# zixinz990/quaternion-mpc

Hardware: AMD Instinct MI355X
Metric: MPC QP solves/sec (Go1, 12 forces, N=10) (higher is better)
Workload: dtype f64

## Files before the change

### quaternion-mpc_amd/csrc/qmpc_wform.h

```cpp
#pragma once

namespace qmpc {


struct LayoutW {
  int GK, WR, SLW;
};
constexpr int kGK = 27;
template <int NL = 4>
__host__ __device__ inline size_t wform_slice(int N, bool sl_global = false) {
  return ((size_t)N * (13 * 12 + 21 * NL + kGK + (sl_global ? 18 * NL : 0)) + 1 + 1) & ~(size_t)1;
}
template <int NL = 4>
__host__ __device__ inline Layout make_layout_w(int N, LayoutW* W, bool kd_global = false, bool sl_global = false, bool cv = false,
                                                bool full = false) {
  Layout L;
  int o = 0;
  auto take = [&](int n) { int r = o; o += n; return r; };
  constexpr int nu = 3 * NL, nc = 6 * NL, nl = NL;
  L.cst = take(NL == 4 ? 64 : 80);
  L.bw0 = take(3 * nu);
  L.refp = take(13);
  L.uref = take(nu);
  L.X = take((N + 1) * 13);
// ... 301 lines not shown
  bool c12;
  template <int NL = 4, int MD = WM_QUAT>
  __device__ __forceinline__ void init(const DevParams& P, const Layout& L, int lane) {
    const int N = P.N;
    const int c = lane & 15, g = lane >> 4;
    co.init(P, c);
    const int zs = L.cst + kZeroSlotsT<NL>();
    const bool c35 = (c >= 3 && c < 6), c911 = (c >= 9 && c < 12);
    c12 = c == 12;
    const int abN = L.AB + kAB * (N - 1);
    ix_w = c35 ? abN + 18 + (c - 3) : zs;   st_w = c35 ? kAB : 0;
    ix_a = c35 ? abN + (c - 3) : (c911 ? abN + 9 + (c - 9) : zs);   st_a = (c35 || c911) ? kAB : 0;
    sel[0] = (g == 3) ? 1.0 : 0.0;
    sel[1] = (g == 0) ? 1.0 : 0.0;
    sel[2] = (g == 1) ? 1.0 : 0.0;
    const double m1 = P.h * (P.hh * (1.0 / P.mass)), m2 = P.h * (1.0 / P.mass);
#pragma unroll
    for (int e = 0; e < 3; ++e) {
      const int r = 4 * e + g;
      const bool phi = (r >= 3 && r < 6);
      double v = 0.0;
      if (c < 6) {
        if (r < 3) v = (r == c) ? m1 : 0.0;
        else if (r >= 6 && r < 9) v = (r - 6 == c) ? m2 : 0.0;
        else if (r >= 9) v = (r - 9 == c - 3) ? P.h : 0.0;
      }
      Mc[e] = v;
      if (MD == WM_CONVEX) qadd[e] = (c < 12 && r == c) ? P.Q[cvperm(r < 12 ? r : 0)] : 0.0;
      else qadd[e] = (c < 12 && r == c && !phi) ? P.Q[(r < 3) ? r : r + 1] : 0.0;
      const bool xv = (MD == WM_CONVEX) ? c12 : ((phi && c35) || c12);
      const int xo = c12 ? 9 + r : 3 * (r - 3) + (c - 3);
      xoffN[e] = xv ? xo : -1;
      ix_x[e] = xv ? L.XT + kXT * (N - 1) + xo : zs;
      st_x[e] = xv ? kXT : 0;
    }
#pragma unroll
    for (int e = 0; e < 2; ++e) {
      const int r = 4 * e + g;
      const bool phi = (r >= 3 && r < 6);
      Nc[e] = (r < 3 && c == r + 6) ? P.h : ((phi && r == c) ? -1.0 : 0.0);
      const bool gv = r < 6 && (c < 6 || c12);
      const int go = c12 ? 21 + r : S6I(r < 6 ? r : 0, c < 6 ? c : 0);
      ix_g[e] = gv ? kGK * (N - 1) + go : kGK * N;
      st_g[e] = gv ? kGK : 0;
      kwo[e] = (r < 6 && c < 13) ? 13 * r + c : -1;
    }
  }
};
__device__ __forceinline__ void fma_bcast345_x2(double r[2], const double x[2], const double sh[2], double cs, const double m[3]) {
  asm("v_fmac_f64 %0, %4, %5\n\t"
      "v_fmac_f64 %1, %4, %6\n\t"
      "v_fmac_f64_dpp %0, %2, %7 row_newbcast:3 row_mask:0xf bank_mask:0xf\n\t"
      "v_fmac_f64_dpp %1, %3, %7 row_newbcast:3 row_mask:0xf bank_mask:0xf\n\t"
      "v_fmac_f64_dpp %0, %2, %8 row_newbcast:4 row_mask:0xf bank_mask:0xf\n\t"
      "v_fmac_f64_dpp %1, %3, %8 row_newbcast:4 row_mask:0xf bank_mask:0xf\n\t"
      "v_fmac_f64_dpp %0, %2, %9 row_newbcast:5 row_mask:0xf bank_mask:0xf\n\t"
      "v_fmac_f64_dpp %1, %3, %9 row_newbcast:5 row_mask:0xf bank_mask:0xf"
      : "+v"(r[0]), "+v"(r[1])
      : "v"(x[0]), "v"(x[1]), "v"(cs), "v"(sh[0]), "v"(sh[1]), "v"(m[0]), "v"(m[1]), "v"(m[2]));
}
__device__ __forceinline__ void fma_bcast345_x3(double r[3], const double x[3], const double sh[3], double cs, const double m[3]) {
  asm("v_fmac_f64 %0, %6, %7\n\t"
      "v_fmac_f64 %1, %6, %8\n\t"
      "v_fmac_f64 %2, %6, %9\n\t"
      "v_fmac_f64_dpp %0, %3, %10 row_newbcast:3 row_mask:0xf bank_mask:0xf\n\t"
      "v_fmac_f64_dpp %1, %4, %10 row_newbcast:3 row_mask:0xf bank_mask:0xf\n\t"
      "v_fmac_f64_dpp %2, %5, %10 row_newbcast:3 row_mask:0xf bank_mask:0xf\n\t"
      "v_fmac_f64_dpp %0, %3, %11 row_newbcast:4 row_mask:0xf bank_mask:0xf\n\t"
      "v_fmac_f64_dpp %1, %4, %11 row_newbcast:4 row_mask:0xf bank_mask:0xf\n\t"
      "v_fmac_f64_dpp %2, %5, %11 row_newbcast:4 row_mask:0xf bank_mask:0xf\n\t"
      "v_fmac_f64_dpp %0, %3, %12 row_newbcast:5 row_mask:0xf bank_mask:0xf\n\t"
      "v_fmac_f64_dpp %1, %4, %12 row_newbcast:5 row_mask:0xf bank_mask:0xf\n\t"
      "v_fmac_f64_dpp %2, %5, %12 row_newbcast:5 row_mask:0xf bank_mask:0xf"
      : "+v"(r[0]), "+v"(r[1]), "+v"(r[2])
      : "v"(x[0]), "v"(x[1]), "v"(x[2]), "v"(cs), "v"(sh[0]), "v"(sh[1]), "v"(sh[2]), "v"(m[0]), "v"(m[1]), "v"(m[2]));
}
__device__ __forceinline__ void times_M(const double x[2], const ColOps& co, const double wt[3], double r[2]) {
  double sh[2];
#pragma unroll
  for (int e = 0; e < 2; ++e) {
    r[e] = co.m1c * x[e];
    sh[e] = dpp_mov<0x106>(x[e]);
  }
  fma_bcast345_x2(r, x, sh, co.m2c, wt);
}
__device__ __forceinline__ void times_Abar(const double x[3], const ColOps& co, const double at[3], double r[3]) {
  double sh[3];
#pragma unroll
  for (int e = 0; e < 3; ++e) {
    r[e] = co.keep * x[e];
    sh[e] = dpp_mov<0x116>(x[e]);
  }
  fma_bcast345_x3(r, x, sh, co.hsel, at);
}

template <int J0, bool INV = false>
__device__ __forceinline__ void gj6_pair_step(double M[2], double Rr[2], double pc[2], int c, int g, bool& pd, double* Iv = nullptr) {
  constexpr int ej = J0 >> 2, g0 = J0 & 3, g1 = g0 + 1;
  static_assert((J0 & 1) == 0 && J0 < 6, "pivot pairs (0,1), (2,3), (4,5)");
  const int s0 = (g0 << 4) | c, s1 = (g1 << 4) | c;
  const double m0 = __shfl(M[ej], s0), m1 = __shfl(M[ej], s1);
  const double r0 = __shfl(Rr[ej], s0), r1 = __shfl(Rr[ej], s1);
  double i0 = 0.0, i1 = 0.0;
  if (INV) { i0 = __shfl(Iv[ej], s0); i1 = __shfl(Iv[ej], s1); }
  const double a = read_lane(M[ej], (g0 << 4) | J0), b = read_lane(M[ej], (g0 << 4) | (J0 + 1)),
               d = read_lane(M[ej], (g1 << 4) | (J0 + 1));
  const double det = fma(a, d, -(b * b));
  pd = pd && (a > 0.0) && (det > 0.0);
  const double rd = fast_rcp(det);
  const double ia = a * rd, ib = b * rd, id = d * rd;
#pragma unroll
  for (int e = 0; e < 2; ++e) {
    double c0, c1;
    double bm = M[e], br = Rr[e], bi = INV ? Iv[e] : 0.0;
    if (e == ej) {
      const bool p0 = g == g0, p1 = g == g1;
      constexpr int others = 0xF & ~((1 << g0) | (1 << g1));
      c0 = pc[0] = row_bcast_rows<J0, others>(M[e], pc[0]);
      c1 = pc[1] = row_bcast_rows<J0 + 1, others>(M[e], pc[1]);
      if (p0 || p1) { bm = 0.0; br = 0.0; bi = 0.0; }
    } else {
      c0 = row_bcast<J0>(M[e]);
      c1 = row_bcast<J0 + 1>(M[e]);
    }
    const double f0 = fma(ib, c1, -(id * c0)), f1 = fma(ib, c0, -(ia * c1));
    M[e] = fma(f1, m1, fma(f0, m0, bm));
    Rr[e] = fma(f1, r1, fma(f0, r0, br));
    if (INV) Iv[e] = fma(f1, i1, fma(f0, i0, bi));
  }
}

template <bool PROF, bool REFINE = false, int MD = WM_QUAT>
__device__ inline int backward_pass_w(const DevParams& P, const Layout& L, const BwPat& bp, double* sm, double* KD,
                                      const double* GK, int lane, Prof<PROF>& prof, double* y0out = nullptr) {
  const int N = P.N;
  const int c = lane & 15, g = lane >> 4;
  const double wscale = (MD == WM_CONVEX) ? P.h * P.hh : (0.5 * P.hh) * P.h;
  const ColOps& co = bp.co;
  const double* Mc = bp.Mc;
  const double* Nc = bp.Nc;
  const double* qadd = bp.qadd;
  const double* msel = bp.sel;
  const double* nsel = bp.sel;
  const int* xoffN = bp.xoffN;
  const int* kwo = bp.kwo;
  int ix_w = bp.ix_w, ix_a = bp.ix_a, ix_x[3] = {bp.ix_x[0], bp.ix_x[1], bp.ix_x[2]}, ix_g[2] = {bp.ix_g[0], bp.ix_g[1]};
  const bool rowok1 = kwo[1] >= 0;
  double Pf[3];
  {
    const double* XTk = sm + L.XT + kXT * N;
#pragma unroll
    for (int e = 0; e < 3; ++e) Pf[e] = qadd[e] + ((xoffN[e] >= 0) ? XTk[xoffN[e]] : 0.0);
  }
  bool pd = true;
  const d4 z4 = {0.0, 0.0, 0.0, 0.0};
  double pc01[2] = {(g == 0) ? 1.0 : 0.0, (g == 1) ? 1.0 : 0.0}, pc23[2] = {(g == 2) ? 1.0 : 0.0, (g == 3) ? 1.0 : 0.0};
  struct KnotOps { double wt[3], at[3], gr[2], xt[3]; };
  auto load_head = [&](KnotOps& o) {
#pragma unroll
    for (int t = 0; t < 3; ++t) o.wt[t] = sm[ix_w + 3 * t];
    ix_w -= bp.st_w;
#pragma unroll
    for (int e = 0; e < 2; ++e) { o.gr[e] = GK[ix_g[e]]; ix_g[e] -= bp.st_g[e]; }
  };
  auto load_tail = [&](KnotOps& o) {
#pragma unroll
    for (int t = 0; t < 3; ++t) {
      o.at[t] = sm[ix_a + 3 * t]; o.xt[t] = sm[ix_x[t]];
      ix_x[t] -= bp.st_x[t];
    }
    ix_a -= bp.st_a;
  };
  KnotOps ops;
  load_head(ops);
  for (int k = N - 1; k >= 0; --k) {
    double wt[3], Mf[3], Nf[2], R6f[2];
    const double* at = ops.at;
    const double* xt = ops.xt;
    const double Gf[2] = {ops.gr[0], ops.gr[1]};
#pragma unroll
    for (int t = 0; t < 3; ++t) wt[t] = wscale * ops.wt[t];
    load_tail(ops);
    Mf[0] = fma(msel[0], wt[0], Mc[0]);
    Mf[1] = fma(msel[1], wt[1], fma(msel[2], wt[2], Mc[1]));
    Mf[2] = Mc[2];
    Nf[0] = fma(nsel[0], at[0], Nc[0]);
    Nf[1] = fma(nsel[1], at[1], fma(nsel[2], at[2], Nc[1]));
    R6f[0] = bp.c12 ? Gf[0] : 0.0;
    R6f[1] = bp.c12 ? Gf[1] : 0.0;
    tick_dep(prof, PH_BUILD, Pf[0], Pf[1]);
    double Yp[2];
    {
      const d4 a = mtm3(Mf, Pf, z4);
      Yp[0] = a[0]; Yp[1] = a[1];
    }
    if (y0out && bp.c12) {
      if (g < 4) y0out[6 * k + g] = Yp[0];
      if (g < 2) y0out[6 * k + 4 + g] = Yp[1];
    }
    tick_dep(prof, PH_DRAIN, Yp[0], Yp[1]);
    double S6[2];
    times_M(Yp, co, wt, S6);
    double Cf[2], Qf[2], Wm[2];
    {
      const d4 a = mtm2(Gf, Yp, acc_rows(R6f[0], R6f[1]));
      Cf[0] = a[0]; Cf[1] = a[1];
      const d4 b = mtm2(S6, Cf, z4);
      Qf[0] = b[0]; Qf[1] = b[1];
    }
    times_M(Qf, co, wt, Wm);
    Wm[0] = S6[0] + Wm[0];
    Wm[1] = S6[1] + Wm[1];
    if (k > 0) load_head(ops);
    tick_dep(prof, PH_MFMA, Wm[0], Wm[1]);
    double Iv[2];
    if (REFINE) {
      Iv[0] = (c == g) ? 1.0 : 0.0;
      Iv[1] = (g < 2 && c == 4 + g) ? 1.0 : 0.0;
    }
    double Xf[2];
    gj6_pair_step<0, REFINE>(Wm, Qf, pc01, c, g, pd, Iv);
    gj6_pair_step<2, REFINE>(Wm, Qf, pc23, c, g, pd, Iv);
    gj6_pair_step<4, REFINE>(Wm, Qf, pc01, c, g, pd, Iv);
    Xf[0] = Qf[0];
    Xf[1] = rowok1 ? Qf[1] : 0.0;
    if (REFINE) {
      double nWi[2], T1[2], nr[2], vv[2];
      nWi[0] = Iv[0];
      nWi[1] = (g < 2) ? Iv[1] : 0.0;
      {
        const d4 a = mtm2(S6, Xf, z4);
        T1[0] = a[0]; T1[1] = a[1];
      }
      {
        const d4 ini = {Cf[0] + Xf[0], Cf[1] + Xf[1], 0.0, 0.0};
        const d4 a = mtm2(Gf, T1, ini);
        nr[0] = a[0]; nr[1] = rowok1 ? a[1] : 0.0;
      }
      {
        const d4 a = mtm2(S6, nr, z4);
        vv[0] = a[0]; vv[1] = a[1];
      }
      {
        const d4 ini = {Xf[0], Xf[1], 0.0, 0.0};
        const d4 a = mtm2(nWi, vv, ini);
        Xf[0] = a[0];
        Xf[1] = rowok1 ? a[1] : 0.0;
      }
    }
    tick_dep(prof, PH_SOLVE, Xf[0], Xf[1]);
    double Pi[3];
    {
      const d4 a = mtm2(Yp, Xf, acc_rows(Pf[0], Pf[1], Pf[2]));
      Pi[0] = a[0]; Pi[1] = a[1]; Pi[2] = a[2];
    }
    double Zf[2];
    {
      const d4 a = mtm2(S6, Xf, acc_rows(Yp[0], Yp[1]));
      Zf[0] = a[0]; Zf[1] = a[1];
    }
    double Uf[3];
    times_Abar(Pi, co, at, Uf);
    {
      const d4 a = mtm2(Nf, Uf, acc_rows(Uf[0] + (qadd[0] + xt[0]), Uf[1] + (qadd[1] + xt[1]), Uf[2] + (qadd[2] + xt[2])));
      Pf[0] = a[0]; Pf[1] = a[1]; Pf[2] = a[2];
    }
    {
      double* KDk = KD + 156 * k;
#pragma unroll
      for (int e = 0; e < 2; ++e) {
        if (kwo[e] >= 0) { KDk[kwo[e]] = Xf[e]; KDk[kwo[e] + 78] = Zf[e]; }
      }
    }
    tick_dep(prof, PH_PUPD, Pf[0], Pf[1]);
  }
  return !pd;
}

__device__ __forceinline__ void srbd_step_w(const DevParams& P, const double gb[3], const double wd0[3], const double* x,
                                            const double w[6], double* xn) {
  double vd[3], wd[3];
#pragma unroll
  for (int a = 0; a < 3; ++a) { vd[a] = w[a] * P.inv_mass + gb[a]; wd[a] = wd0[a] + w[3 + a]; }
  double G[12];
  quat_G(&x[3], G);
  double qm[4], wm[3];
#pragma unroll
  for (int r = 0; r < 4; ++r)
    qm[r] = x[3 + r] + P.hh * (0.5 * (G[3 * r] * x[10] + G[3 * r + 1] * x[11] + G[3 * r + 2] * x[12]));
#pragma unroll
  for (int a = 0; a < 3; ++a) wm[a] = x[10 + a] + P.hh * wd[a];
  quat_G(qm, G);
#pragma unroll
  for (int a = 0; a < 3; ++a) {
    xn[a] = x[a] + P.h * (x[7 + a] + P.hh * vd[a]);
    xn[7 + a] = x[7 + a] + P.h * vd[a];
    xn[10 + a] = x[10 + a] + P.h * wd[a];
  }
#pragma unroll
  for (int r = 0; r < 4; ++r)
    xn[3 + r] = x[3 + r] + P.h * (0.5 * (G[3 * r] * wm[0] + G[3 * r + 1] * wm[1] + G[3 * r + 2] * wm[2]));
}

template <bool WITH_DU, int NL = 4, bool ONEW = false>
__device__ inline void wrench_from_inputs(const DevParams& P, const Layout& L, const LayoutW& LW, double* sm, int lane) {
  const int N = P.N;
  constexpr int NU = 3 * NL;
  for (int q = lane; q < 6 * N; q += kWave) {
    const int k = q / 6, i = q - 6 * k;
    double u[NU];
    double u0[NU], du0[NU], b0[NU];
    if constexpr (ONEW) {
#pragma unroll
      for (int j = 0; j < NU; ++j) {
        u0[j] = sm[L.U + NU * k + j];
        if (WITH_DU) du0[j] = sm[L.dU + NU * k + j];
        b0[j] = sm[L.bw0 + ((i >= 3) ? NU * (i - 3) : 0) + j];
      }
      __builtin_amdgcn_sched_barrier(0);
#pragma unroll
      for (int j = 0; j < NU; ++j) u[j] = u0[j] + (WITH_DU ? du0[j] : 0.0);
    } else {
#pragma unroll
    for (int j = 0; j < NU; ++j) u[j] = sm[L.U + NU * k + j] + (WITH_DU ? sm[L.dU + NU * k + j] : 0.0);
    }
    const double* b = ONEW ? b0 : sm + L.bw0 + ((i >= 3) ? NU * (i - 3) : 0);
    if (NL == 4) {
      double s0 = 0.0, s1 = 0.0, f0 = 0.0, f1 = 0.0;
#pragma unroll
      for (int j = 0; j < 6; ++j) { s0 += b[j] * u[j]; s1 += b[6 + j] * u[6 + j]; }
#pragma unroll
      for (int a = 0; a < 3; ++a) {
        f0 += (i == a) ? u[a] + u[6 + a] : 0.0;
        f1 += (i == a) ? u[3 + a] + u[9 + a] : 0.0;
      }
      sm[LW.WR + q] = (i < 3) ? f0 + f1 : s0 + s1;
    } else {
      double sv[4] = {0.0, 0.0, 0.0, 0.0}, fv[4] = {0.0, 0.0, 0.0, 0.0};
#pragma unroll
      for (int j = 0; j < NU; ++j) sv[j / 6] += b[j] * u[j];
#pragma unroll
      for (int l = 0; l < NL; ++l)
#pragma unroll
        for (int a = 0; a < 3; ++a) fv[l >> 1] += (i == a) ? u[3 * l + a] : 0.0;
      sm[LW.WR + q] = (i < 3) ? (fv[0] + fv[1]) + (fv[2] + fv[3]) : (sv[0] + sv[1]) + (sv[2] + sv[3]);
    }
  }
  QSYNC();
}

template <int NL = 4, int MD = WM_QUAT, bool ONEW = false>
__device__ inline void rollout_scaled_w(const DevParams& P, const Layout& L, const LayoutW& LW, double* sm, double ap, int lane) {
  typedef Dim<NL> D;
  const int N = P.N;
  const double* cst = sm + L.cst;
  for (int i = lane; i < N * D::NU; i += kWave) sm[L.dU + i] *= ap;
  QSYNC();
  wrench_from_inputs<true, NL, ONEW>(P, L, LW, sm, lane);
  double gb[3], wd0[3];
#pragma unroll
  for (int a = 0; a < 3; ++a) { gb[a] = cst[D::C_GB + a]; wd0[a] = cst[D::C_WD0 + a]; }
  double x[13], xn[13], w[6], wn[6];
#pragma unroll
  for (int i = 0; i < 13; ++i) x[i] = cst[D::C_X0 + i];
#pragma unroll
  for (int i = 0; i < 6; ++i) w[i] = sm[LW.WR + i];
  for (int k = 0; k < N; ++k) {
    const int kn = (k + 1 < N) ? k + 1 : k;
#pragma unroll
    for (int i = 0; i < 6; ++i) wn[i] = sm[LW.WR + 6 * kn + i];
    if (MD == WM_CONVEX) cv_step_w(P, x, w, xn);
    else srbd_step_w(P, gb, wd0, x, w, xn);
#pragma unroll
    for (int i = 0; i < 13; ++i) x[i] = xn[i];
#pragma unroll
    for (int i = 0; i < 6; ++i) w[i] = wn[i];
    if (lane == 0)
#pragma unroll
      for (int i = 0; i < 13; ++i) sm[L.Xc + 13 * (k + 1) + i] = xn[i];
  }
  QSYNC();
}

template <int NL = 4, int MD = WM_QUAT>
__device__ inline void expansions_w(const DevParams& P, const Layout& L, const LayoutW& LW, double* sm, int lane) {
  typedef Dim<NL> D;
  const int N = P.N;
  const double* cst = sm + L.cst;
  if (MD == WM_CONVEX) {
    for (int k = lane; k <= N; k += kWave) {
      double x[12];
#pragma unroll
      for (int i = 0; i < 12; ++i) x[i] = sm[L.X + 13 * k + i];
      double* ABk = sm + L.AB + kAB * k;
      double* XTk = sm + L.XT + kXT * k;
      if (k < N) {
        const double t0 = sm[LW.WR + 6 * k + 3], t1 = sm[LW.WR + 6 * k + 4];
        double s0, c0, w00, w01, w11;
        sincos(x[2], &s0, &c0);
        ConvexModel::winv(P, c0, s0, w00, w01, w11);
        const double wm0 = x[6] + P.hh * (w00 * t0 + w01 * t1);
        const double wm1 = x[7] + P.hh * (w01 * t0 + w11 * t1);
        double sm_, cm_;
        sincos(x[2] + P.hh * x[8], &sm_, &cm_);
        const double j0 = wm1 * cm_ - wm0 * sm_, j1 = -wm0 * cm_ - wm1 * sm_;
        const double m00 = cm_ * w00 + sm_ * w01, m01 = cm_ * w01 + sm_ * w11;
        const double m10 = -sm_ * w00 + cm_ * w01, m11 = -sm_ * w01 + cm_ * w11;
        ConvexModel::winv(P, cm_, sm_, w00, w01, w11);
        const double ixx = 1.0 / P.Iinv[0], iyy = 1.0 / P.Iinv[4], izz = 1.0 / P.Iinv[8];
        const double i00 = cm_ * cm_ * ixx + sm_ * sm_ * iyy, i01 = cm_ * sm_ * (ixx - iyy), i11 = sm_ * sm_ * ixx + cm_ * cm_ * iyy;
        ABk[0] = 1.0; ABk[1] = 0.0; ABk[2] = P.h * j0;
        ABk[3] = 0.0; ABk[4] = 1.0; ABk[5] = P.h * j1;
        ABk[6] = 0.0; ABk[7] = 0.0; ABk[8] = 1.0;
        ABk[9] = P.h * cm_;   ABk[10] = P.h * sm_; ABk[11] = P.h * P.hh * j0;
        ABk[12] = -P.h * sm_; ABk[13] = P.h * cm_; ABk[14] = P.h * P.hh * j1;
        ABk[15] = 0.0; ABk[16] = 0.0; ABk[17] = P.h;
        ABk[18] = m00 * i00 + m01 * i01; ABk[19] = m00 * i01 + m01 * i11; ABk[20] = 0.0;
        ABk[21] = m10 * i00 + m11 * i01; ABk[22] = m10 * i01 + m11 * i11; ABk[23] = 0.0;
        ABk[24] = 0.0; ABk[25] = 0.0; ABk[26] = 1.0;
        double* CVk = sm + L.CV + 8 * k;
        CVk[0] = w00; CVk[1] = w01; CVk[2] = w11; CVk[3] = P.Iinv[8];
        CVk[4] = i00; CVk[5] = i01; CVk[6] = i11; CVk[7] = izz;
      }
#pragma unroll
      for (int i = 0; i < 9; ++i) XTk[i] = 0.0;
      double xr[12];
      ConvexModel::xref(P, sm + L.refp, k, xr);
#pragma unroll
      for (int r = 0; r < 12; ++r) XTk[9 + r] = P.Q[cvperm(r)] * (x[cvperm(r)] - xr[cvperm(r)]);
    }
    QSYNC();
    return;
  }
  for (int q = lane; q < 4 * (N + 1); q += kWave) {
    const int k = q >> 2, part = q & 3;
    double x[13];
#pragma unroll
    for (int i = 0; i < 13; ++i) x[i] = sm[L.X + 13 * k + i];
    double* ABk = sm + L.AB + kAB * k;
    double* XTk = sm + L.XT + kXT * k;
    if (part < 3) {
      if (k >= N) continue;
      const int c = part;
      double xn[4], wd[3];
#pragma unroll
      for (int i = 0; i < 4; ++i) xn[i] = sm[L.X + 13 * (k + 1) + 3 + i];
#pragma unroll
      for (int a = 0; a < 3; ++a) wd[a] = cst[D::C_WD0 + a] + sm[LW.WR + 6 * k + 3 + a];
      double G0[12], Gm[12], Gn[12];
      quat_G(&x[3], G0);
      double qm[4], wm[3];
#pragma unroll
      for (int r = 0; r < 4; ++r)
        qm[r] = x[3 + r] + P.hh * (0.5 * (G0[3 * r] * x[10] + G0[3 * r + 1] * x[11] + G0[3 * r + 2] * x[12]));
#pragma unroll
      for (int a = 0; a < 3; ++a) wm[a] = x[10 + a] + P.hh * wd[a];
      quat_G(qm, Gm);
      quat_G(xn, Gn);
      double g[4], gm[4];
#pragma unroll
      for (int r = 0; r < 4; ++r) {
        g[r] = (c == 0) ? G0[3 * r] : (c == 1 ? G0[3 * r + 1] : G0[3 * r + 2]);
        gm[r] = (c == 0) ? Gm[3 * r] : (c == 1 ? Gm[3 * r + 1] : Gm[3 * r + 2]);
      }
      double t0[4], t1[4], t2[4], ag[4], aw[4];
      omega_mul(&x[10], g, t0);
#pragma unroll
      for (int r = 0; r < 4; ++r) t1[r] = g[r] + (0.5 * P.hh) * t0[r];
      omega_mul(wm, t1, t2);
      omega_mul(wm, g, t0);
#pragma unroll
      for (int r = 0; r < 4; ++r) {
        ag[r] = g[r] + P.hh * t2[r];
        aw[r] = P.hh * ((0.5 * P.hh) * t0[r] + gm[r]);
      }
#pragma unroll
      for (int r = 0; r < 3; ++r) {
        ABk[3 * r + c] = Gn[r] * ag[0] + Gn[3 + r] * ag[1] + Gn[6 + r] * ag[2] + Gn[9 + r] * ag[3];
        ABk[9 + 3 * r + c] = Gn[r] * aw[0] + Gn[3 + r] * aw[1] + Gn[6 + r] * aw[2] + Gn[9 + r] * aw[3];
        ABk[18 + 3 * r + c] = Gn[r] * gm[0] + Gn[3 + r] * gm[1] + Gn[6 + r] * gm[2] + Gn[9 + r] * gm[3];
      }
    } else {
      double u0[1] = {0.0};
      expand_knot_part<NL>(P, cst, sm + L.bw0, sm + L.refp, k, 3, x, u0, x, ABk, XTk);
    }
  }
  QSYNC();
}

struct RollLoadsW {
  double xo[13], ab[18], kd[13], wk;
};
struct RollLoadsC {
  double wr[6], iw[4];
};
__device__ __forceinline__ void roll_load_c(const Layout& L, const LayoutW& LW, const double* sm, int k, RollLoadsC& r) {
#pragma unroll
  for (int i = 0; i < 6; ++i) r.wr[i] = sm[LW.WR + 6 * k + i];
#pragma unroll
  for (int i = 0; i < 4; ++i) r.iw[i] = sm[L.CV + 8 * k + 4 + i];
}
__device__ __forceinline__ void roll_load_state(const Layout& L, const double* sm, int k, RollLoadsW& r) {
#pragma unroll
  for (int i = 0; i < 13; ++i) r.xo[i] = sm[L.X + 13 * k + i];
#pragma unroll
  for (int i = 0; i < 18; ++i) r.ab[i] = sm[L.AB + kAB * k + i];
}
__device__ __forceinline__ void roll_load_gains(const LayoutW& LW, const double* sm, const double* KD, int k, int row, int wi,
                                                RollLoadsW& r) {
  const double* kd = KD + 156 * k + 13 * row;
#pragma unroll
  for (int i = 0; i < 13; ++i) r.kd[i] = kd[i];
  r.wk = sm[LW.WR + 6 * k + wi];
}
template <bool PROF, bool PF, int NL = 4, int MD = WM_QUAT, bool BC = false>
__device__ inline void rollout_closed_w(const DevParams& P, const Layout& L, const LayoutW& LW, double* sm,
                                        const double* KD, double* ROT, int lane, Prof<PROF>& prof, double alpha = 1.0) {
  typedef Dim<NL> D;
  const int N = P.N;
  const double* cst = sm + L.cst;
  double gb[3], wd0[3];
#pragma unroll
  for (int a = 0; a < 3; ++a) { gb[a] = cst[D::C_GB + a]; wd0[a] = cst[D::C_WD0 + a]; }
  const int row = (lane < 12) ? lane : 0, wi = (lane < 6) ? lane : 0;
  const bool zlane = lane >= 6 && lane < 12;
  double xc[13], xn[13];
#pragma unroll
  for (int i = 0; i < 13; ++i) xc[i] = cst[D::C_X0 + i];
  if (lane == 0)
#pragma unroll
    for (int i = 0; i < 13; ++i) sm[L.Xc + i] = xc[i];
  auto knot = [&](int k, RollLoadsW& cur, RollLoadsW& nxt) {
    roll_load_state(L, sm, k, cur);
    if (!PF) roll_load_gains(LW, sm, KD, k, row, wi, cur);
    double dx[12], e[12];
    if (MD == WM_CONVEX) {
#pragma unroll
      for (int r = 0; r < 12; ++r) dx[r] = xc[cvperm(r)] - cur.xo[cvperm(r)];
    } else {
      QuatModel::state_diff(cur.xo, xc, dx);
    }
#pragma unroll
    for (int a = 0; a < 3; ++a) {
      e[a] = dx[a] + P.h * dx[6 + a];
      e[3 + a] = (cur.ab[3 * a] * dx[3] + cur.ab[3 * a + 1] * dx[4] + cur.ab[3 * a + 2] * dx[5]) +
                 (cur.ab[9 + 3 * a] * dx[9] + cur.ab[9 + 3 * a + 1] * dx[10] + cur.ab[9 + 3 * a + 2] * dx[11]);
      e[6 + a] = dx[6 + a];
      e[9 + a] = dx[9 + a];
    }
    const double* kd = cur.kd;
    const double p0 = alpha * kd[12] + kd[0] * e[0] + kd[1] * e[1] + kd[2] * e[2];
    const double p1 = kd[3] * e[3] + kd[4] * e[4] + kd[5] * e[5];
    const double p2 = kd[6] * e[6] + kd[7] * e[7] + kd[8] * e[8];
    const double p3 = kd[9] * e[9] + kd[10] * e[10] + kd[11] * e[11];
    const double s = (p0 + p1) + (p2 + p3);
    if (zlane) ROT[zeta_slot<NL>(k, lane - 6)] = s;
    double wn = (MD == WM_CONVEX) ? s : cur.wk + s;
    tick_dep1(prof, PH_R_GAIN, wn);
    if (PF && k + 1 < N) roll_load_gains(LW, sm, KD, k + 1, row, wi, nxt);
    double w[6];
    if (BC) {
      w[0] = row_bcast<0>(wn); w[1] = row_bcast<1>(wn); w[2] = row_bcast<2>(wn);
      w[3] = row_bcast<3>(wn); w[4] = row_bcast<4>(wn); w[5] = row_bcast<5>(wn);
    } else {
#pragma unroll
    for (int i = 0; i < 6; ++i) w[i] = read_lane(wn, i);
    }
    tick_dep(prof, PH_R_BCAST, w[0], w[5]);
    if (MD == WM_CONVEX) {
      RollLoadsC rc;
      roll_load_c(L, LW, sm, k, rc);
      const double d3 = rc.iw[0] * w[3] + rc.iw[1] * w[4], d4 = rc.iw[1] * w[3] + rc.iw[2] * w[4], d5 = rc.iw[3] * w[5];
      w[0] += rc.wr[0]; w[1] += rc.wr[1]; w[2] += rc.wr[2];
      w[3] = rc.wr[3] + d3; w[4] = rc.wr[4] + d4; w[5] = rc.wr[5] + d5;
      cv_step_w(P, xc, w, xn);
    } else
    srbd_step_w(P, gb, wd0, xc, w, xn);
#pragma unroll
    for (int i = 0; i < 13; ++i) xc[i] = xn[i];
    if (lane == 0)
#pragma unroll
      for (int i = 0; i < 13; ++i) sm[L.Xc + 13 * (k + 1) + i] = xn[i];
    tick_dep(prof, PH_R_STEP, xc[3], xc[10]);
  };
  if (PF) {
    RollLoadsW ra, rb;
    roll_load_gains(LW, sm, KD, 0, row, wi, ra);
    for (int k = 0; k < N; k += 2) {
      knot(k, ra, rb);
      if (k + 1 < N) knot(k + 1, rb, ra);
    }
  } else {
    RollLoadsW ra;
    for (int k = 0; k < N; ++k) knot(k, ra, ra);
  }
  QSYNC();
}

template <int MD = WM_QUAT, int NL = 4>
__device__ inline double expected_decrease_w(const DevParams& P, const Layout& L, double* sm, const double* KD,
                                             const double* ROT, const double* y0, int lane) {
  typedef Dim<NL> D;
  constexpr int LSH = (NL == 8) ? 3 : 2;
  const int N = P.N;
  const double* cst = sm + L.cst;
  double part = 0.0;
  for (int q = lane; q < NL * N; q += kWave) {
    const int k = q >> LSH, l = q & (NL - 1);
    if (cst[D::C_CON + l] == 0.0) continue;
    const double* rec = ROT + D::ROT * k + 21 * l;
    double T[9], xz[6], yk[6];
#pragma unroll
    for (int i = 0; i < 9; ++i) T[i] = rec[i];
#pragma unroll
    for (int i = 0; i < 6; ++i) { xz[i] = KD[156 * k + 13 * (6 + i) + 12]; yk[i] = y0[6 * k + i]; }
    if (MD == WM_CONVEX) {
      double a[3], b[3];
      cv_winv_mul(sm + L.CV + 8 * k, xz + 3, a);
      cv_winv_mul(sm + L.CV + 8 * k, yk + 3, b);
#pragma unroll
      for (int i = 0; i < 3; ++i) { xz[3 + i] = a[i]; yk[3 + i] = b[i]; }
    }
    const double l10 = rec[9], l20 = rec[10], l21 = rec[11], id0 = rec[12], id1 = rec[13], id2 = rec[14];
    const double* bw = sm + L.bw0 + 3 * l;
    double fz[3], fy[3];
#pragma unroll
    for (int b = 0; b < 3; ++b) {
      fz[b] = xz[b] + (bw[b] * xz[3] + bw[D::NU + b] * xz[4] + bw[2 * D::NU + b] * xz[5]);
      fy[b] = yk[b] + (bw[b] * yk[3] + bw[D::NU + b] * yk[4] + bw[2 * D::NU + b] * yk[5]);
    }
    double t[3], qu[3];
#pragma unroll
    for (int b = 0; b < 3; ++b) {
      t[b] = rec[15 + b] + (T[b] * fz[0] + T[3 + b] * fz[1] + T[6 + b] * fz[2]);
      qu[b] = rec[15 + b] + (T[b] * fy[0] + T[3 + b] * fy[1] + T[6 + b] * fy[2]);
    }
    const double y0_ = t[0], y1_ = t[1] - l10 * y0_, y2_ = t[2] - l20 * y0_ - l21 * y1_;
    const double x2 = id2 * y2_;
    const double x1 = id1 * y1_ - l21 * x2;
    const double x0 = id0 * y0_ - l10 * x1 - l20 * x2;
    part -= x0 * qu[0] + x1 * qu[1] + x2 * qu[2];
  }
  return wave_sum(part);
}

template <int NL = 4, int MD = WM_QUAT>
__device__ inline int recover_inputs_w(const DevParams& P, const Layout& L, double* sm, const double* ROT, int lane,
                                       double alpha = 1.0, const double* zsrc = nullptr) {
  typedef Dim<NL> D;
  constexpr int LSH = (NL == 8) ? 3 : 2;
  const int N = P.N;
  const double* cst = sm + L.cst;
  bool bad = false;
  for (int q = lane; q < NL * N; q += kWave) {
    const int k = q >> LSH, l = q & (NL - 1);
    double du[3] = {0.0, 0.0, 0.0};
    if (cst[D::C_CON + l] != 0.0) {
      const double* rec = ROT + D::ROT * k + 21 * l;
      double T[9], z[6];
#pragma unroll
      for (int i = 0; i < 9; ++i) T[i] = rec[i];
#pragma unroll
      for (int i = 0; i < 6; ++i) z[i] = zsrc ? zsrc[6 * k + i] : ROT[zeta_slot<NL>(k, i)];
      if (MD == WM_CONVEX) {
        double y[3];
        cv_winv_mul(sm + L.CV + 8 * k, z + 3, y);
        z[3] = y[0]; z[4] = y[1]; z[5] = y[2];
      }
      const double l10 = rec[9], l20 = rec[10], l21 = rec[11], id0 = rec[12], id1 = rec[13], id2 = rec[14];
      const double* bw = sm + L.bw0 + 3 * l;
      double f[3];
#pragma unroll
      for (int b = 0; b < 3; ++b) f[b] = z[b] + (bw[b] * z[3] + bw[D::NU + b] * z[4] + bw[2 * D::NU + b] * z[5]);
      double t[3];
#pragma unroll
      for (int b = 0; b < 3; ++b) t[b] = alpha * rec[15 + b] + (T[b] * f[0] + T[3 + b] * f[1] + T[6 + b] * f[2]);
      const double y0 = t[0], y1 = t[1] - l10 * y0, y2 = t[2] - l20 * y0 - l21 * y1;
      const double x2 = id2 * y2;
      const double x1 = id1 * y1 - l21 * x2;
      const double x0 = id0 * y0 - l10 * x1 - l20 * x2;
#pragma unroll
      for (int a = 0; a < 3; ++a) du[a] = -(T[3 * a] * x0 + T[3 * a + 1] * x1 + T[3 * a + 2] * x2);
    }
    double* o = sm + L.dU + D::NU * k + 3 * l;
    o[0] = du[0]; o[1] = du[1]; o[2] = du[2];
    bad = bad || !(isfinite(du[0]) && isfinite(du[1]) && isfinite(du[2]));
  }
  QSYNC();
  return __any(bad ? 1 : 0);
}

template <int NL = 4, int MD = WM_QUAT, bool LEAN = (NL == 8), bool ONEW = false>
__device__ inline int recover_directions_w(const DevParams& P, const Layout& L, double* sm, double* sl, const double* ROT,
                                           double target, int lane, double* alpha_p, double* alpha_d, double* full_step,
                                           unsigned& kapbits) {
  typedef Dim<NL> D;
  constexpr int LSH = (NL == 8) ? 3 : 2;
  const int N = P.N;
  const double* cst = sm + L.cst;
  double cr0[18], bw0[2 * D::NU + 3];
  const double* cr = ONEW ? cr0 : cst + D::C_CR;
  bool bad = false;
  double pn = 1.0, pd = 0.0, dn = 1.0, dd = 0.0;
  double stp = 0.0;
  unsigned bits = 0;
  int j = 0;
  for (int q = lane; q < NL * N; q += kWave, ++j) {
    const int k = q >> LSH, l = q & (NL - 1);
    const bool stance = cst[D::C_CON + l] != 0.0;
    const double* rec = ROT + D::ROT * k + 21 * l;
    const int i0 = D::NC * k + 6 * l;
    double T[9], z[6], sv[6], lv[6], kap[6], rc[6];
#pragma unroll
    for (int i = 0; i < 9; ++i) T[i] = rec[i];
#pragma unroll
    for (int i = 0; i < 6; ++i) z[i] = ROT[zeta_slot<NL>(k, i)];
    if (MD == WM_CONVEX) {
      double y[3];
      if (ONEW) cv_winv_mul_dirs(sm + L.CV + 8 * k, z + 3, y);
      else
      cv_winv_mul(sm + L.CV + 8 * k, z + 3, y);
      z[3] = y[0]; z[4] = y[1]; z[5] = y[2];
    }
    const double l10 = rec[9], l20 = rec[10], l21 = rec[11], id0 = rec[12], id1 = rec[13], id2 = rec[14];
    const double g0 = rec[15], g1 = rec[16], g2 = rec[17];
#pragma unroll
    for (int i = 0; i < 6; ++i) {
      sv[i] = sl[L.S + i0 + i]; lv[i] = sl[L.LAM + i0 + i]; rc[i] = sl[L.RC + i0 + i];
      kap[i] = LEAN ? (((kapbits >> (6 * j + i)) & 1u) ? 1.0 : 0.0) : sl[L.DS + i0 + i];
    }
    const double* bw = sm + L.bw0 + 3 * l;
    if constexpr (ONEW) {
#pragma unroll
      for (int a = 0; a < 3; ++a)
#pragma unroll
        for (int b = 0; b < 3; ++b) bw0[D::NU * a + b] = bw[D::NU * a + b];
      __builtin_amdgcn_sched_barrier(0);
      bw = bw0;
    }
    double du[3] = {0.0, 0.0, 0.0};
    if (stance) {
      double f[3];
#pragma unroll
      for (int b = 0; b < 3; ++b) f[b] = z[b] + (bw[b] * z[3] + bw[D::NU + b] * z[4] + bw[2 * D::NU + b] * z[5]);
      const double t0 = g0 + (T[0] * f[0] + T[3] * f[1] + T[6] * f[2]);
      const double t1 = g1 + (T[1] * f[0] + T[4] * f[1] + T[7] * f[2]);
      const double t2 = g2 + (T[2] * f[0] + T[5] * f[1] + T[8] * f[2]);
      const double y0 = t0, y1 = t1 - l10 * y0, y2 = t2 - l20 * y0 - l21 * y1;
      const double x2 = id2 * y2;
      const double x1 = id1 * y1 - l21 * x2;
      const double x0 = id0 * y0 - l10 * x1 - l20 * x2;
#pragma unroll
      for (int a = 0; a < 3; ++a) du[a] = -(T[3 * a] * x0 + T[3 * a + 1] * x1 + T[3 * a + 2] * x2);
    }
    if constexpr (ONEW) {
#pragma unroll
      for (int i = 0; i < 18; ++i) cr0[i] = cst[D::C_CR + i];
    }
    double* o = sm + L.dU + D::NU * k + 3 * l;
    o[0] = du[0]; o[1] = du[1]; o[2] = du[2];
    bad = bad || !(isfinite(du[0]) && isfinite(du[1]) && isfinite(du[2]));
    stp = fmax(stp, fmax(fabs(du[0]), fmax(fabs(du[1]), fabs(du[2]))));
    if constexpr (ONEW) __builtin_amdgcn_sched_barrier(0);
#pragma unroll
    for (int i = 0; i < 6; ++i) {
      const double jd = cr[3 * i] * du[0] + cr[3 * i + 1] * du[1] + cr[3 * i + 2] * du[2];
      double dsv = -(jd + rc[i]);
      double dlv = (target - (1.0 + kap[i]) * sv[i] * lv[i] - lv[i] * dsv) * fast_rcp(sv[i]);
      dsv = stance ? dsv : 0.0;
      dlv = stance ? dlv : 0.0;
      const bool up = (int)(dsv < 0.0) & ((int)(pd == 0.0) | (int)(sv[i] * pd < pn * (-dsv)));
      pn = up ? sv[i] : pn; pd = up ? -dsv : pd;
      const bool ud = (int)(dlv < 0.0) & ((int)(dd == 0.0) | (int)(lv[i] * dd < dn * (-dlv)));
      dn = ud ? lv[i] : dn; dd = ud ? -dlv : dd;
      if (!LEAN) {
        sl[L.DS + i0 + i] = dsv;
        sl[L.DLAM + i0 + i] = dlv;
      }
      bits |= (stance && kap[i] != 0.0) ? (1u << (6 * j + i)) : 0u;
    }
  }
  const double ap = (pd > 0.0) ? fmin(1.0, P.tau * pn * fast_rcp(pd)) : 1.0;
  const double ad = (dd > 0.0) ? fmin(1.0, P.tau * dn * fast_rcp(dd)) : 1.0;
  *alpha_p = wave_min(ap);
  *alpha_d = wave_min(ad);
  *full_step = wave_max(stp);
  kapbits = bits;
  QSYNC();
  return __any(bad ? 1 : 0);
}

template <int NL = 4, bool LEAN = (NL == 8)>
__device__ inline void apply_w(const DevParams& P, const Layout& L, double* sl, double ap, double ad, unsigned conmask,
                               int lane, unsigned& kapbits, double& sl_part, double& rc_part, const double* sm = nullptr,
                               double target = 0.0) {
  typedef Dim<NL> D;
  constexpr int LSH = (NL == 8) ? 3 : 2;
  const int N = P.N;
  sl_part = 0.0;
  rc_part = 0.0;
  const bool full = (ap >= 0.99) && (ad >= 0.99);
  const double rcs = (ap >= 1.0) ? 0.0 : (1.0 - ap);
  int j = 0;
  for (int q = lane; q < NL * N; q += kWave, ++j) {
    const int k = q >> LSH, l = q & (NL - 1);
    if (!(conmask & (1u << l))) continue;
    const int i0 = D::NC * k + 6 * l;
    double s0[6], l0[6], ds[6], dl[6], rc[6];
#pragma unroll
    for (int i = 0; i < 6; ++i) {
      s0[i] = sl[L.S + i0 + i]; l0[i] = sl[L.LAM + i0 + i]; rc[i] = sl[L.RC + i0 + i];
      if (!LEAN) { ds[i] = sl[L.DS + i0 + i]; dl[i] = sl[L.DLAM + i0 + i]; }
    }
    if (LEAN) {
      const double* cr = sm + L.cst + D::C_CR;
      const double* du = sm + L.dU + D::NU * k + 3 * l;
      const double du0 = du[0], du1 = du[1], du2 = du[2];
#pragma unroll
      for (int i = 0; i < 6; ++i) {
        const double kp = ((kapbits >> (6 * j + i)) & 1u) ? 1.0 : 0.0;
        const double jd = cr[3 * i] * du0 + cr[3 * i + 1] * du1 + cr[3 * i + 2] * du2;
        ds[i] = -(jd + rc[i]);
        dl[i] = (target - (1.0 + kp) * s0[i] * l0[i] - l0[i] * ds[i]) * fast_rcp(s0[i]);
      }
    }
    unsigned newbits = 0;
#pragma unroll
    for (int i = 0; i < 6; ++i) {
// ... 238 lines not shown
```

### quaternion-mpc_amd/csrc/qmpc_wform_body.inc

```
#ifndef QMPC_WNL
#define QMPC_WNL 4
#define QMPC_WNL_DEFAULTED 1
#endif
#ifndef QMPC_WMODEL
#define QMPC_WMODEL WM_QUAT
#define QMPC_WMODEL_DEFAULTED 1
#endif
  constexpr int WNL = QMPC_WNL;
  constexpr int WMT = QMPC_WMODEL;
  typedef typename std::conditional<WMT == WM_CONVEX, ConvexModel, QuatModelT<WNL>>::type WMD;
  typedef Dim<WNL> WD;
  constexpr int NU = WD::NU, NC = WD::NC;
  const int N = P.N;
  constexpr bool KDG = WVAR == 5 || WVAR == 6;
  constexpr bool SLG = WVAR == 6;
  constexpr bool LEAN = WNL == 8 || SLG;
  LayoutW LW;
  const Layout L = make_layout_w<WNL>(N, &LW, KDG, SLG, WMT == WM_CONVEX);
  double* wsb = KDG ? gws + (size_t)wslot * wform_slice<WNL>(N, SLG) : sm;
  double* KD = wsb + L.KD;
  double* ROT = wsb + L.ROT;
  double* GK = wsb + LW.GK;
  double* sl = SLG ? wsb + LW.SLW : sm;
  const void* in = reinterpret_cast<const double*>(in_) + (size_t)b * WD::REC;
  int status = QMPC_OK;
  Prof<PROF> prof;
  prof.start();
  setup_instance<WMD>(P, L, sm, in, lane, &status);
  if (status != QMPC_OK) {
    if (lane < NU) forces[NU * (size_t)b + lane] = 0.0;
    if (lane == 0 && info) {
      qmpc_info r = {status, 0, 0.0, 0.0, 0.0, 0.0};
      info[b] = r;
    }
    if (traj_u) for (int i = lane; i < N * NU; i += kWave) traj_u[(size_t)b * N * NU + i] = 0.0;
    if (traj_x) for (int i = lane; i < (N + 1) * WMD::NX; i += kWave) traj_x[(size_t)b * (N + 1) * WMD::NX + i] = 0.0;
    return;
  }
  unsigned conmask = 0;
  for (int l = 0; l < WMD::NL; ++l) conmask |= (sm[L.cst + WD::C_CON + l] != 0.0) ? (1u << l) : 0u;
  conmask = __builtin_amdgcn_readfirstlane(conmask);
  if (lane < 10) sm[L.cst + kZeroSlotsT<WNL>() + lane] = 0.0;
  if (lane == 0) GK[kGK * N] = 0.0;
  BwPat bp;
  if (!KDG) bp.init<WNL, WMT>(P, L, lane);
  if (resume) {
    for (int i = lane; i < N * NU; i += kWave) sm[L.U + i] = resume[8 + i];
  } else if (warm_t > 0) {
    if (lane < NU) {
      const bool stance = (conmask >> (lane / 3)) & 1u;
      for (int k = 0; k < N; ++k) {
        const double prev = sm[L.U + ((k + 1 < N) ? k + 1 : k) * NU + lane];
        sm[L.U + k * NU + lane] = !stance ? 0.0 : (prev != 0.0 ? prev : sm[L.uref + lane]);
      }
    }
  } else {
    for (int i = lane; i < N * NU; i += kWave) sm[L.U + i] = sm[L.uref + (i % NU)];
  }
  QSYNC();
  rollout_open<WMD, false>(P, L, sm, lane);
  wrench_from_inputs<false, WNL, !KDG>(P, L, LW, sm, lane);
  expansions_w<WNL, WMT>(P, L, LW, sm, lane);
  double sl_part = 0.0, rc_part = 0.0;
  unsigned kapbits = 0;
  if (resume) {
    const double rho = resume[0];
    int j = 0;
    for (int i = lane; i < N * NC; i += kWave, ++j) {
      const int row = i % NC, l = row / 6, r = row - 6 * l;
      const double* cr = sm + L.cst + WD::C_CR + 3 * r;
      const double* ur = sm + L.uref + 3 * l;
      double c0 = cr[0] * ur[0] + cr[1] * ur[1] + cr[2] * ur[2];
      if (r == 4) c0 += -P.fz_max * sm[L.cst + WD::C_CON + l];
      const double s0 = fmax(-c0, 1.0);
      const double sraw = resume[8 + N * NU + i], lam = resume[8 + N * NU + N * NC + i];
      const double sv = fabs(sraw), rc = rho * ((resume[5] != 0.0) ? resume[8 + N * NU + 2 * N * NC + i] : (c0 + s0));
      const bool flag = sraw < 0.0;
      sl[L.S + i] = sv;
      sl[L.RC + i] = rc;
      sl[L.LAM + i] = lam;
      if (!LEAN) sl[L.DS + i] = flag ? 1.0 : 0.0;
      if (conmask & (1u << l)) {
        sl_part += sv * lam;
        rc_part = fmax(rc_part, fabs(rc));
        kapbits |= flag ? (1u << j) : 0u;
      }
    }
  } else
  for (int i = lane; i < N * NC; i += kWave) {
    const double c0 = cone_value<WD>(P, L, sm, i);
    const double s0 = fmax(-c0, 1.0);
    const double lam0 = P.mu0 / s0;
    sl[L.S + i] = s0;
    sl[L.RC + i] = c0 + s0;
    sl[L.LAM + i] = lam0;
    if (!LEAN) sl[L.DS + i] = 0.0;
    if (conmask & (1u << ((i % NC) / 6))) {
      sl_part += s0 * lam0;
      rc_part = fmax(rc_part, fabs(c0 + s0));
    }
  }
  QSYNC();
  prof.tick(PH_SETUP);
  const double inv_rows = 1.0 / (double)(6 * N * __popc(conmask));
  const int it_start = resume ? (int)resume[4] + 1 : 1;
  int it = 0, iters = it_start - 1;
  double mu = 0.0, resid = 0.0, last_step = resume ? resume[3] : 1e300, last_ap = resume ? resume[1] : 0.0,
         last_ad = resume ? resume[2] : 0.0;
  status = QMPC_MAX_ITER;
  mu = wave_sum(sl_part) * inv_rows;
  resid = wave_max(rc_part);
  for (it = it_start; it <= P.iterations_max + 1; ++it) {
    if (mu <= P.mu_final && resid <= P.tol_feas && last_step <= P.tol_step) { status = QMPC_OK; break; }
    if (it > P.iterations_max) break;
    double sg = P.sigma;
    const double amin = fmin(last_ap, last_ad);
    if (it > 1 && amin >= 0.99) sg = P.sigma_fast;
    else if (it > 1 && amin < 0.2) sg = fmax(sg, 0.8);
    else if (it > 1 && amin < 0.5) sg = fmax(sg, 0.5);
    const double target = sg * mu;
    prof.tick(PH_MISC);
    prepass_w<false, WNL, WMT, LEAN>(P, L, sm, sl, ROT, GK, target, lane, kapbits);
    prof.tick(PH_PREPASS);
    if (KDG) bp.init<WNL, WMT>(P, L, lane);
    if (backward_pass_w<PROF, false, WMT>(P, L, bp, sm, KD, GK, lane, prof)) { status = QMPC_NOT_PD; break; }
    QSYNC();
    double ap, ad;
    rollout_closed_w<PROF, !KDG, WNL, WMT, !KDG>(P, L, LW, sm, KD, ROT, lane, prof);
    prof.tick(PH_ROLL);
    {
      double stp_;
      if (recover_directions_w<WNL, WMT, LEAN, !KDG>(P, L, sm, sl, ROT, target, lane, &ap, &ad, &stp_, kapbits)) { status = QMPC_NOT_PD; break; }
      last_step = stp_;
    }
    last_ap = ap; last_ad = ad;
    prof.tick(PH_DIRS);
    if (LEAN) apply_w<WNL, true>(P, L, sl, ap, ad, conmask, lane, kapbits, sl_part, rc_part, sm, target);
    if (ap < 1.0) rollout_scaled_w<WNL, WMT, !KDG>(P, L, LW, sm, ap, lane);
    prof.tick(PH_ROLL);
    if (!LEAN) apply_w<WNL, false>(P, L, sl, ap, ad, conmask, lane, kapbits, sl_part, rc_part);
    prof.tick(PH_APPLY);
    for (int i = lane; i < N * NU; i += kWave) sm[L.U + i] += sm[L.dU + i];
    for (int i = lane; i < (N + 1) * 13; i += kWave) sm[L.X + i] = sm[L.Xc + i];
    QSYNC();
    iters = it;
    mu = wave_sum(sl_part) * inv_rows;
    resid = wave_max(rc_part);
    if ((mu <= P.mu_final && resid <= P.tol_feas && last_step <= P.tol_step) || it >= P.iterations_max) continue;
    if (!(ap < 1.0)) wrench_from_inputs<false, WNL, !KDG>(P, L, LW, sm, lane);
    prof.tick(PH_MISC);
    expansions_w<WNL, WMT>(P, L, LW, sm, lane);
    prof.tick(PH_EXPAND);
  }
  if (lane < NU) forces[NU * (size_t)b + lane] = sm[L.U + lane];
  if (traj_u) for (int i = lane; i < N * NU; i += kWave) traj_u[(size_t)b * N * NU + i] = sm[L.U + i];
  if (traj_x)
    for (int i = lane; i < (N + 1) * WMD::NX; i += kWave) {
      if (WMD::NX == 13) {
        traj_x[(size_t)b * (N + 1) * WMD::NX + i] = sm[L.X + i];
      } else {
        const int k_ = i / WMD::NX, j_ = i - WMD::NX * k_;
        traj_x[(size_t)b * (N + 1) * WMD::NX + i] = sm[L.X + 13 * k_ + j_];
      }
    }
  if (info) {
    const double J = cost_plain<WMD>(P, L, sm, lane);
    double viol = 0.0;
    for (int i = lane; i < N * NC; i += kWave) {
      const int l = (i % NC) / 6;
      if (conmask & (1u << l)) viol = fmax(viol, fmax(cone_value<WD>(P, L, sm, i), 0.0));
    }
    viol = wave_max(viol);
    if (lane == 0) {
      qmpc_info r = {status, iters, J, viol, last_step, mu};
      info[b] = r;
    }
  }
  if (PROF && prof_out && lane == 0) {
    prof.tick(PH_MISC);
#pragma unroll
    for (int i = 0; i < PH_COUNT; ++i) prof_out[16 * (size_t)b + i] = prof.t[i];
    prof_out[16 * (size_t)b + 15] = iters;
  }
#ifdef QMPC_WMODEL_DEFAULTED
#undef QMPC_WMODEL
#undef QMPC_WMODEL_DEFAULTED
#endif
#ifdef QMPC_WNL_DEFAULTED
#undef QMPC_WNL
#undef QMPC_WNL_DEFAULTED
#endif
```

Before: 2.115 million.

## Split closed-loop and scaled rollouts across lanes with per-axis state

Adds a lane-distributed form of the closed-loop rollout and the scaled rollout for the quaternion model. Each lane now carries only its own position and velocity axis plus the shared quaternion and angular rate, instead of every lane integrating the full 13-state. The state error and wrench components are shared between lanes with row broadcasts, and the quaternion products are rewritten as pinned FMA chains. The goal is to shorten the serial per-knot dependency chain and cut redundant per-lane arithmetic, in exchange for more cross-lane broadcasts and a possible change in floating-point rounding.

```diff
diff --git a/quaternion-mpc_amd/csrc/qmpc_wform.h b/quaternion-mpc_amd/csrc/qmpc_wform.h
--- a/quaternion-mpc_amd/csrc/qmpc_wform.h
+++ b/quaternion-mpc_amd/csrc/qmpc_wform.h
@@ -627,6 +627,101 @@
     xn[3 + r] = x[3 + r] + P.h * (0.5 * (G[3 * r] * wm[0] + G[3 * r + 1] * wm[1] + G[3 * r + 2] * wm[2]));
 }
 
+__device__ __forceinline__ double flip_sign(double x, int m) {
+  return __hiloint2double(__double2hiint(x) ^ m, __double2loint(x));
+}
+__device__ __forceinline__ void quat_G_mul_pinned(const double q[4], const double w[3], double d[4]) {
+#pragma clang fp contract(off)
+  const double s = q[0], x = q[1], y = q[2], z = q[3];
+  d[0] = fma(-w[2], z, fma(w[1], -y, -(w[0] * x)));
+  d[1] = fma(w[2], y, fma(w[0], s, -(w[1] * z)));
+  d[2] = fma(-w[2], x, fma(w[0], z, w[1] * s));
+  d[3] = fma(w[2], s, fma(w[1], x, -(w[0] * y)));
+}
+struct RollLoadsL {
+  double qo[4], wo[3], po, vo, g[4], ab[6];
+};
+struct LanePat {
+  int a, iq[4], ms[4];
+  __device__ __forceinline__ void init(int lane) {
+    const int c = lane & 15;
+    a = (c < 3) ? c : 0;
+    iq[0] = a + 1;
+    iq[1] = (a == 0) ? 0 : ((a == 1) ? 3 : 2);
+    iq[2] = (a == 0) ? 3 : ((a == 1) ? 0 : 1);
+    iq[3] = 2 - a;
+    const int sb = (int)0x80000000u;
+    ms[0] = 0; ms[1] = (a == 1) ? sb : 0; ms[2] = (a == 2) ? sb : 0; ms[3] = (a == 0) ? sb : 0;
+  }
+};
+__device__ __forceinline__ void roll_load_lane(const Layout& L, const double* sm, int k, const LanePat& lp, RollLoadsL& r) {
+  const double* xk = sm + L.X + 13 * k;
+  const double* abk = sm + L.AB + kAB * k + 3 * lp.a;
+#pragma unroll
+  for (int i = 0; i < 4; ++i) r.qo[i] = xk[3 + i];
+#pragma unroll
+  for (int i = 0; i < 3; ++i) r.wo[i] = xk[10 + i];
+  r.po = xk[lp.a];
+  r.vo = xk[7 + lp.a];
+#pragma unroll
+  for (int t = 0; t < 4; ++t) r.g[t] = xk[3 + lp.iq[t]];
+#pragma unroll
+  for (int j = 0; j < 3; ++j) { r.ab[j] = abk[j]; r.ab[3 + j] = abk[9 + j]; }
+}
+__device__ __forceinline__ double roll_gain_lane(double h, const double q[4], const double om[3], double S, double V,
+                                                 const RollLoadsL& r, const LanePat& lp, const double kd[13], double alpha) {
+#pragma clang fp contract(off)
+  const double isc = fast_rcp(fma(q[3], r.qo[3], fma(q[2], r.qo[2], fma(q[0], r.qo[0], q[1] * r.qo[1]))));
+  const double g1 = flip_sign(r.g[1], lp.ms[1]), g2 = flip_sign(r.g[2], lp.ms[2]), g3 = flip_sign(r.g[3], lp.ms[3]);
+  const double d = fma(q[3], g3, fma(q[2], g2, fma(q[1], g1, -(q[0] * r.g[0])))) * isc;
+  double e[12];
+#pragma unroll
+  for (int i = 0; i < 3; ++i) e[9 + i] = om[i] - r.wo[i];
+  const double dp = S - r.po, dv = V - r.vo;
+  const double e0 = fma(h, dv, dp);
+  const double d3 = row_bcast<0>(d), d4 = row_bcast<1>(d), d5 = row_bcast<2>(d);
+  const double e3 = fma(r.ab[2], d5, fma(r.ab[0], d3, r.ab[1] * d4)) + fma(r.ab[5], e[11], fma(r.ab[3], e[9], r.ab[4] * e[10]));
+  e[0] = row_bcast<0>(e0); e[1] = row_bcast<1>(e0); e[2] = row_bcast<2>(e0);
+  e[3] = row_bcast<0>(e3); e[4] = row_bcast<1>(e3); e[5] = row_bcast<2>(e3);
+  e[6] = row_bcast<0>(dv); e[7] = row_bcast<1>(dv); e[8] = row_bcast<2>(dv);
+  const double p0 = fma(kd[2], e[2], fma(kd[1], e[1], fma(kd[0], e[0], alpha * kd[12])));
+  const double p1 = fma(kd[5], e[5], fma(kd[3], e[3], kd[4] * e[4]));
+  const double p2 = fma(kd[8], e[8], fma(kd[6], e[6], kd[7] * e[7]));
+  const double p3 = fma(kd[11], e[11], fma(kd[9], e[9], kd[10] * e[10]));
+  return (p0 + p1) + (p2 + p3);
+}
+__device__ __forceinline__ void roll_step_lane(const DevParams& P, double gba, const double wd0[3], double wf, const double wt[3],
+                                               double q[4], double om[3], double& S, double& V) {
+#pragma clang fp contract(off)
+  double wd[3], wm[3], d[4], qm[4];
+#pragma unroll
+  for (int i = 0; i < 3; ++i) wd[i] = wd0[i] + wt[i];
+  const double vd = fma(P.inv_mass, wf, gba);
+  quat_G_mul_pinned(q, om, d);
+#pragma unroll
+  for (int r = 0; r < 4; ++r) qm[r] = fma(P.hh, d[r] * 0.5, q[r]);
+#pragma unroll
+  for (int i = 0; i < 3; ++i) wm[i] = fma(P.hh, wd[i], om[i]);
+  quat_G_mul_pinned(qm, wm, d);
+#pragma unroll
+  for (int r = 0; r < 4; ++r) q[r] = fma(P.h, d[r] * 0.5, q[r]);
+#pragma unroll
+  for (int i = 0; i < 3; ++i) om[i] = fma(P.h, wd[i], om[i]);
+  const double t = fma(P.hh, vd, V);
+  S = fma(P.h, t, S);
+  V = fma(P.h, vd, V);
+}
+__device__ __forceinline__ void roll_store_lane(double* xk, int lane, const double q[4], const double om[3], double S, double V) {
+  if (lane < 3) {
+    xk[lane] = S;
+    xk[7 + lane] = V;
+#pragma unroll
+    for (int r = 0; r < 4; ++r) xk[3 + r] = q[r];
+#pragma unroll
+    for (int i = 0; i < 3; ++i) xk[10 + i] = om[i];
+  }
+}
+
 template <bool WITH_DU, int NL = 4, bool ONEW = false>
 __device__ inline void wrench_from_inputs(const DevParams& P, const Layout& L, const LayoutW& LW, double* sm, int lane) {
   const int N = P.N;
@@ -685,6 +780,31 @@
   double gb[3], wd0[3];
 #pragma unroll
   for (int a = 0; a < 3; ++a) { gb[a] = cst[D::C_GB + a]; wd0[a] = cst[D::C_WD0 + a]; }
+  if constexpr (ONEW && MD != WM_CONVEX) {
+    LanePat lp;
+    lp.init(lane);
+    const double gba = cst[D::C_GB + lp.a];
+    double q[4], om[3], wt[3], wtn[3];
+    double S = cst[D::C_X0 + lp.a], V = cst[D::C_X0 + 7 + lp.a];
+#pragma unroll
+    for (int i = 0; i < 4; ++i) q[i] = cst[D::C_X0 + 3 + i];
+#pragma unroll
+    for (int i = 0; i < 3; ++i) { om[i] = cst[D::C_X0 + 10 + i]; wt[i] = sm[LW.WR + 3 + i]; }
+    double wf = sm[LW.WR + lp.a];
+    for (int k = 0; k < N; ++k) {
+      const int kn = (k + 1 < N) ? k + 1 : k;
+      const double wfn = sm[LW.WR + 6 * kn + lp.a];
+#pragma unroll
+      for (int i = 0; i < 3; ++i) wtn[i] = sm[LW.WR + 6 * kn + 3 + i];
+      roll_step_lane(P, gba, wd0, wf, wt, q, om, S, V);
+      wf = wfn;
+#pragma unroll
+      for (int i = 0; i < 3; ++i) wt[i] = wtn[i];
+      roll_store_lane(sm + L.Xc + 13 * (k + 1), lane, q, om, S, V);
+    }
+    QSYNC();
+    return;
+  }
   double x[13], xn[13], w[6], wn[6];
 #pragma unroll
   for (int i = 0; i < 13; ++i) x[i] = cst[D::C_X0 + i];
@@ -838,7 +958,7 @@
   for (int i = 0; i < 13; ++i) r.kd[i] = kd[i];
   r.wk = sm[LW.WR + 6 * k + wi];
 }
-template <bool PROF, bool PF, int NL = 4, int MD = WM_QUAT, bool BC = false>
+template <bool PROF, bool PF, int NL = 4, int MD = WM_QUAT, bool BC = false, bool LN = false>
 __device__ inline void rollout_closed_w(const DevParams& P, const Layout& L, const LayoutW& LW, double* sm,
                                         const double* KD, double* ROT, int lane, Prof<PROF>& prof, double alpha = 1.0) {
   typedef Dim<NL> D;
@@ -849,6 +969,42 @@
   for (int a = 0; a < 3; ++a) { gb[a] = cst[D::C_GB + a]; wd0[a] = cst[D::C_WD0 + a]; }
   const int row = (lane < 12) ? lane : 0, wi = (lane < 6) ? lane : 0;
   const bool zlane = lane >= 6 && lane < 12;
+  if constexpr (LN && MD != WM_CONVEX) {
+    static_assert(PF && BC, "the lane form belongs to the all-LDS form with one wave per SIMD");
+    LanePat lp;
+    lp.init(lane);
+    const double gba = cst[D::C_GB + lp.a];
+    double q[4], om[3];
+    double S = cst[D::C_X0 + lp.a], V = cst[D::C_X0 + 7 + lp.a];
+#pragma unroll
+    for (int i = 0; i < 4; ++i) q[i] = cst[D::C_X0 + 3 + i];
+#pragma unroll
+    for (int i = 0; i < 3; ++i) om[i] = cst[D::C_X0 + 10 + i];
+    roll_store_lane(sm + L.Xc, lane, q, om, S, V);
+    auto knot = [&](int k, RollLoadsW& cur, RollLoadsW& nxt) {
+      RollLoadsL rl;
+      roll_load_lane(L, sm, k, lp, rl);
+      const double s = roll_gain_lane(P.h, q, om, S, V, rl, lp, cur.kd, alpha);
+      if (zlane) ROT[zeta_slot<NL>(k, lane - 6)] = s;
+      double wn = cur.wk + s;
+      tick_dep1(prof, PH_R_GAIN, wn);
+      if (k + 1 < N) roll_load_gains(LW, sm, KD, k + 1, row, wi, nxt);
+      double wt[3];
+      wt[0] = row_bcast<3>(wn); wt[1] = row_bcast<4>(wn); wt[2] = row_bcast<5>(wn);
+      tick_dep(prof, PH_R_BCAST, wt[0], wt[2]);
+      roll_step_lane(P, gba, wd0, wn, wt, q, om, S, V);
+      roll_store_lane(sm + L.Xc + 13 * (k + 1), lane, q, om, S, V);
+      tick_dep(prof, PH_R_STEP, q[0], om[0]);
+    };
+    RollLoadsW ra, rb;
+    roll_load_gains(LW, sm, KD, 0, row, wi, ra);
+    for (int k = 0; k < N; k += 2) {
+      knot(k, ra, rb);
+      if (k + 1 < N) knot(k + 1, rb, ra);
+    }
+    QSYNC();
+    return;
+  }
   double xc[13], xn[13];
 #pragma unroll
   for (int i = 0; i < 13; ++i) xc[i] = cst[D::C_X0 + i];
diff --git a/quaternion-mpc_amd/csrc/qmpc_wform_body.inc b/quaternion-mpc_amd/csrc/qmpc_wform_body.inc
--- a/quaternion-mpc_amd/csrc/qmpc_wform_body.inc
+++ b/quaternion-mpc_amd/csrc/qmpc_wform_body.inc
@@ -126,7 +126,7 @@
     if (backward_pass_w<PROF, false, WMT>(P, L, bp, sm, KD, GK, lane, prof)) { status = QMPC_NOT_PD; break; }
     QSYNC();
     double ap, ad;
-    rollout_closed_w<PROF, !KDG, WNL, WMT, !KDG>(P, L, LW, sm, KD, ROT, lane, prof);
+    rollout_closed_w<PROF, !KDG, WNL, WMT, !KDG, !KDG>(P, L, LW, sm, KD, ROT, lane, prof);
     prof.tick(PH_ROLL);
     {
       double stp_;
```

Result: faster. 2.201 million (median of 6 runs) (+4.1%).
